# soedinglab/spacedust

Hardware: AMD Instinct MI355X
Metric: clustersearch throughput (genome-pairs/s; SW GCUPS alongside) (higher is better)
Workload: dtype int16

## Files before the change

### spacedust_amd/csrc/hip/sd_sw.hip

```cpp
#include "sd_common.h"
#include <unistd.h>


#include <algorithm>
#include <cmath>
#include <cstring>
#include <memory>
#include <omp.h>
#include <numeric>

#include "../host/sd_host.h"
#include "sd_sw_pk.h"

namespace {

using sdpk::SwTask;

template <int RT>
__global__ void __launch_bounds__(64)
sw_score_kernel(const SwTask *__restrict__ tasks, uint32_t nTasks, const uint8_t *__restrict__ qRes,
                const int8_t *__restrict__ qBias, const uint8_t *__restrict__ tRes, const int8_t *__restrict__ mat,
                int go, int ge, int32_t *__restrict__ out, uint2 *__restrict__ boundary,
                const uint32_t *__restrict__ order ,
                const int8_t *__restrict__ qProf ) {
// ... 804 lines not shown
    }
    SD_HIP(ctx, hipMemcpyAsync(hPin, dOut, (size_t) nSlots * 3 * sizeof(int32_t), hipMemcpyDeviceToHost, ctx->stream));
    SD_HIP(ctx, sdStreamSync(ctx));
    memcpy(hOut.data(), hPin, (size_t) nSlots * 3 * sizeof(int32_t));
    return SD_OK;
}


constexpr uint32_t N_NARROW_CLASSES = 24;
constexpr uint32_t FIRST_NARROW_MULTI = 21;
constexpr uint32_t N_PK_CLASSES = 14;
constexpr uint32_t FIRST_MULTI_PK = 11;
constexpr uint32_t FIRST_WIDE_CLASS = N_NARROW_CLASSES;
constexpr uint32_t FIRST_INT32_CLASS = FIRST_WIDE_CLASS + N_PK_CLASSES;
constexpr uint32_t N_SCORE_CLASSES = FIRST_INT32_CLASS + 4;
static_assert(N_SCORE_CLASSES < 63, "class boundaries are found by one 64-lane wavefront; six class bits in the pair key");
enum ScoreKernel { SCORE_PK = 0, SCORE_PK_WIDE = 1, SCORE_INT32 = 2 };
constexpr uint32_t KEY_INVALID = N_SCORE_CLASSES * 1024u;
__host__ __device__ __forceinline__ bool scoreClassIsMulti(uint32_t ci) {
    return (ci >= FIRST_NARROW_MULTI && ci < FIRST_WIDE_CLASS) || (ci >= FIRST_WIDE_CLASS + FIRST_MULTI_PK && ci < FIRST_INT32_CLASS);
}
__device__ __forceinline__ uint32_t scoreKey(int n, int tL, int kernel, int wideRowLimit = 800) {
    int ci;
    if (kernel == SCORE_PK_WIDE && min(n, tL) > wideRowLimit) kernel = SCORE_INT32;
    if (kernel == SCORE_INT32 || tL > 65535) {
        ci = FIRST_INT32_CLASS + (n <= 128 ? 0 : (n <= 256 ? 1 : (n <= 512 ? 2 : 3)));
    } else if (kernel == SCORE_PK_WIDE) {
        if (n <= 192) ci = n <= 128 ? 0 : 1;
        else if (n <= 384) ci = 2 + (n - 193) / 32;
        else if (n <= 768) ci = n <= 512 ? 8 : (n <= 640 ? 9 : 10);
        else ci = min((int) FIRST_MULTI_PK + (n + 511) / 512 - 2, 13);
        ci += FIRST_WIDE_CLASS;
    } else {
        if (n <= 128) ci = 0;
        else if (n <= 768) ci = (n + 31) / 32 - 4;
        else ci = min((int) FIRST_NARROW_MULTI + (n + 511) / 512 - 2, (int) FIRST_WIDE_CLASS - 1);
    }
    return (uint32_t) ci * 1024u + (uint32_t) (1023 - min(tL >> 4, 1023));
}

struct DevGateParams {
    int go, ge, matMin, swMode, covMode, wideRowLimit;
    float covThr;
    double evalThr;
    double lambda, K, aI, bI, alphaI, betaI, aJ, bJ, alphaJ, betaJ, sigma, tau, viThr, vjThr, cThr, dbResidues;
};

__device__ double devEvalue(const DevGateParams &e, double y_, double qLen) {
    const double m_ = e.dbResidues, n_ = qLen;
    const double const_val = 0.3989422804014327;
    double tmp = e.aI * y_ + e.bI;
    double m_li_y = m_ - tmp;
    double vi_y = fmax(e.viThr, e.alphaI * y_ + e.betaI);
    double sqrt_vi_y = sqrt(vi_y);
    double m_F = sqrt_vi_y == 0.0 ? 1e100 : m_li_y / sqrt_vi_y;
    double P_m_F = 0.5 * erfc(-sqrt(0.5) * m_F);
    double E_m_F = -const_val * exp(-0.5 * m_F * m_F);
    double p1 = m_li_y * P_m_F - sqrt_vi_y * E_m_F;
    tmp = e.aJ * y_ + e.bJ;
    double n_lj_y = n_ - tmp;
    double vj_y = fmax(e.vjThr, e.alphaJ * y_ + e.betaJ);
    double sqrt_vj_y = sqrt(vj_y);
    double n_F = sqrt_vj_y == 0.0 ? 1e100 : n_lj_y / sqrt_vj_y;
    double P_n_F = 0.5 * erfc(-sqrt(0.5) * n_F);
    double E_n_F = -const_val * exp(-0.5 * n_F * n_F);
    double p2 = n_lj_y * P_n_F - sqrt_vj_y * E_n_F;
    double c_y = fmax(e.cThr, e.sigma * y_ + e.tau);
    double area = p1 * p2 + c_y * (P_m_F * P_n_F);
    return e.K * exp(-e.lambda * y_) * area;
}

__device__ __forceinline__ float devCov(unsigned int startPos, unsigned int endPos, unsigned int len) {
    return (min(len, max(startPos, endPos)) - min(startPos, endPos) + 1) / (float) len;
}
__device__ __forceinline__ bool devHasCoverage(float covThr, int covMode, float qCov, float tCov) {
    switch (covMode) {
        case 0: return (qCov >= covThr) && (tCov >= covThr);
        case 2: return qCov >= covThr;
        case 1: return tCov >= covThr;
        default: return true;
    }
}

__global__ void __launch_bounds__(256)
k_pre_word(uint32_t nPairs, const uint32_t *__restrict__ pairQ, const uint32_t *__restrict__ pairT, const uint16_t *__restrict__ pairDiag,
           const uint32_t *__restrict__ fwdKeys, const uint64_t *__restrict__ qOff, const uint64_t *__restrict__ tOff,
           const uint8_t *__restrict__ qRes, const int8_t *__restrict__ qBias, const uint8_t *__restrict__ tRes, const int8_t *__restrict__ mat,
           const int8_t *__restrict__ qProf, const int32_t *__restrict__ minBias, int matMin, uint8_t *__restrict__ preWord,
           uint32_t *__restrict__ pass1Keys) {
    __shared__ int8_t smat[441];
    for (int x = threadIdx.x; x < 441; x += blockDim.x) smat[x] = mat[x];
    __syncthreads();
    const uint32_t i = blockIdx.x * blockDim.x + threadIdx.x;
    if (i >= nPairs) return;
    uint8_t pw = 0;
    const uint32_t key = fwdKeys[i];
    if (key != KEY_INVALID) {
        const uint64_t qo = qOff[pairQ[i]], to = tOff[pairT[i]];
        const int qL = (int) (qOff[pairQ[i] + 1] - qo), tL = (int) (tOff[pairT[i] + 1] - to);
        if (qL < 32768 && tL < 32768 && pairDiag[i] != 0x8000) {
            const int d = (int) (int16_t) pairDiag[i];
            int q0 = d >= 0 ? d : 0, t0 = d >= 0 ? 0 : -d;
            const int n = min(qL - q0, tL - t0);
            const int need = 255 - (abs(matMin) + abs(minBias[pairQ[i]]));
            int run = 0, best = 0;
            for (int x = 0; x < n && best < need; x++) {
                const int qr = qRes[qo + q0 + x], tr = tRes[to + t0 + x];
                run += qProf ? (int) qProf[(qo + q0 + x) * 21 + tr] : (int) smat[tr * 21 + qr] + (int) qBias[qo + q0 + x];
                run = run < 0 ? 0 : run;
                best = run > best ? run : best;
            }
            pw = best >= need ? 1 : 0;
        }
    }
    preWord[i] = pw;
    pass1Keys[i] = pw ? KEY_INVALID : key;
}

__global__ void __launch_bounds__(256)
k_make_fwd(uint32_t nPairs, const uint32_t *__restrict__ pairQ, const uint32_t *__restrict__ pairT,
           const uint8_t *__restrict__ ident, const uint64_t *__restrict__ qOff, const uint64_t *__restrict__ tOff,
           SwTask *__restrict__ tasks, uint32_t *__restrict__ keys, uint32_t *__restrict__ vals,
           sd_sw_result *__restrict__ res, int usePk) {
    const uint32_t i = blockIdx.x * blockDim.x + threadIdx.x;
    if (i >= nPairs) return;
    const uint64_t qo = qOff[pairQ[i]], to = tOff[pairT[i]];
    const int qL = (int) (qOff[pairQ[i] + 1] - qo), tL = (int) (tOff[pairT[i] + 1] - to);
    SwTask tk;
    tk.qOff = qo; tk.tOff = to; tk.n = qL; tk.tL = tL; tk.qStep = 1; tk.tStep = 1;
    tk.segLen = max(1, (qL + 31) / 32);
    tk.slot = i; tk.boundOff = 0;
    const bool valid = !(ident && ident[i]) && qL > 0 && tL > 0;
    tasks[i] = tk;
    keys[i] = valid ? scoreKey(qL, tL, usePk ? SCORE_PK : SCORE_INT32) : KEY_INVALID;
    vals[i] = i;
    sd_sw_result r;
    r.score = 0; r.qStart = -1; r.qEnd = -1; r.tStart = -1; r.tEnd = -1; r.identical = 0; r.btLen = 0; r.flags = 0;
    r.evalue = 0.0; r.btOffset = 0;
    res[i] = r;
}

__global__ void k_bounds(const uint32_t *__restrict__ keys, uint32_t n, uint32_t step, uint32_t *__restrict__ b, int nb) {
    const int c = threadIdx.x;
    if (c >= nb) return;
    const uint64_t want = (uint64_t) c * step;
    uint32_t lo = 0, hi = n;
    while (lo < hi) {
        uint32_t mid = (lo + hi) >> 1;
        if ((uint64_t) keys[mid] < want) lo = mid + 1;
        else hi = mid;
    }
    b[c] = lo;
}

__global__ void __launch_bounds__(256)
k_gate_word(uint32_t nPairs, const uint32_t *__restrict__ pairQ, const int32_t *__restrict__ out32,
            const int32_t *__restrict__ minBias, int matMin, SwTask *__restrict__ tasks, uint32_t *__restrict__ keys,
            uint32_t *__restrict__ vals, uint8_t *__restrict__ word, const uint32_t *__restrict__ fwdKeys, int usePk, int wideRowLimit,
            const uint8_t *__restrict__ preWord ) {
    const uint32_t i = blockIdx.x * blockDim.x + threadIdx.x;
    if (i >= nPairs) return;
    vals[i] = i;
    bool w = false;
    if (fwdKeys[i] != KEY_INVALID) {
        const int mb = minBias[pairQ[i]];
        const int bias = abs(matMin) + abs(mb);
        w = (preWord && preWord[i]) || out32[3 * i] + bias >= 255;
    }
    word[i] = w ? 1 : 0;
    if (w) {
        tasks[i].segLen = max(1, (tasks[i].n + 15) / 16);
        keys[i] = scoreKey(tasks[i].n, tasks[i].tL, usePk ? SCORE_PK_WIDE : SCORE_INT32, wideRowLimit);
    } else {
        keys[i] = KEY_INVALID;
    }
}

__global__ void __launch_bounds__(256)
k_gate_rev(uint32_t nPairs, DevGateParams gp, const uint32_t *__restrict__ pairQ, const uint32_t *__restrict__ pairT,
           const uint64_t *__restrict__ qOff, const uint64_t *__restrict__ tOff, const int32_t *__restrict__ out32,
           const int32_t *__restrict__ out16, const uint8_t *__restrict__ word, const uint32_t *__restrict__ fwdKeys,
           SwTask *__restrict__ tasks, uint32_t *__restrict__ keys, uint32_t *__restrict__ vals,
           sd_sw_result *__restrict__ res, int usePk) {
    const uint32_t i = blockIdx.x * blockDim.x + threadIdx.x;
    if (i >= nPairs) return;
    vals[i] = i;
    keys[i] = KEY_INVALID;
    if (fwdKeys[i] == KEY_INVALID) return;
    const int32_t *src = word[i] ? &out16[3 * i] : &out32[3 * i];
    sd_sw_result r = res[i];
    r.score = src[0];
    r.tEnd = src[1];
    r.qEnd = src[2];
    r.flags = word[i] ? 1 : 0;
    if (word[i] && r.tEnd == -1) r.tEnd = 0;
    if (r.score == 0) r.qEnd = 0;
    if (r.tEnd == -1) { res[i] = r; return; }
    const uint64_t qo = qOff[pairQ[i]], to = tOff[pairT[i]];
    const int qL = (int) (qOff[pairQ[i] + 1] - qo), tL = (int) (tOff[pairT[i] + 1] - to);
// ... 918 lines not shown
    std::unique_ptr<HostScope> hs(new HostScope(ctx, "align.upload"));
    DevGateParams gp;
    gp.go = go; gp.ge = ge; gp.matMin = matMin; gp.swMode = par->swMode; gp.covMode = par->covMode; gp.covThr = par->covThr;
    {
        int matMax = 0;
        for (int x = 0; x < 441; x++) matMax = std::max(matMax, (int) par->matrix[x]);
        const int maxEntry = std::max(1, queries->dProf ? queries->maxEntryAdd : matMax + queries->maxEntryAdd);
        gp.wideRowLimit = 32767 / maxEntry;
    }
    gp.evalThr = par->evalThr;
    gp.lambda = ev.lambda; gp.K = ev.K; gp.aI = ev.aI; gp.bI = ev.bI; gp.alphaI = ev.alphaI; gp.betaI = ev.betaI;
    gp.aJ = ev.aJ; gp.bJ = ev.bJ; gp.alphaJ = ev.alphaJ; gp.betaJ = ev.betaJ; gp.sigma = ev.sigma; gp.tau = ev.tau;
    gp.viThr = ev.viThr; gp.vjThr = ev.vjThr; gp.cThr = ev.cThr; gp.dbResidues = ev.dbResidues;

    const size_t N = nPairs;
    const unsigned grid = (unsigned) ((N + 255) / 256);
    int8_t *dMat = nullptr;
    uint32_t *dPQ = nullptr, *dPT = nullptr, *dKeys = nullptr, *dVals = nullptr, *dKeysS = nullptr, *dOrder = nullptr,
             *dBounds = nullptr, *dFwdKeys = nullptr, *dRevKeys = nullptr;
    uint8_t *dIdent = nullptr, *dWord = nullptr;
    int32_t *dMinBias = nullptr, *dOut32 = nullptr, *dOut16 = nullptr, *dOutRev = nullptr, *dTbRes = nullptr;
    int *dErr = nullptr;
    SwTask *dTasks = nullptr;
    TbTask *dTb = nullptr;
    sd_sw_result *dRes = nullptr;
    uint64_t *dScanA = nullptr, *dScanB = nullptr, *dDirBytes = nullptr, *dDirOff = nullptr, *dBtBytes = nullptr,
             *dBtOff = nullptr, *dBtLen = nullptr, *dDense = nullptr;
    unsigned long long *dCells = nullptr;
    SD_HIP(ctx, wsGet(ctx, "al.mat", 448, &dMat));
    SD_HIP(ctx, wsGet(ctx, "al.pq", N, &dPQ));
    SD_HIP(ctx, wsGet(ctx, "al.pt", N, &dPT));
    SD_HIP(ctx, wsGet(ctx, "al.ident", N, &dIdent));
    SD_HIP(ctx, wsGet(ctx, "al.word", N, &dWord));
    SD_HIP(ctx, wsGet(ctx, "al.keys", N, &dKeys));
    SD_HIP(ctx, wsGet(ctx, "al.vals", N, &dVals));
    SD_HIP(ctx, wsGet(ctx, "al.keyss", N, &dKeysS));
    SD_HIP(ctx, wsGet(ctx, "al.order", N, &dOrder));
    SD_HIP(ctx, wsGet(ctx, "al.fwdkeys", N, &dFwdKeys));
    SD_HIP(ctx, wsGet(ctx, "al.revkeys", N, &dRevKeys));
    SD_HIP(ctx, wsGet(ctx, "al.bounds", 64, &dBounds));
    SD_HIP(ctx, wsGet(ctx, "al.minbias", queries->n, &dMinBias));
    SD_HIP(ctx, wsGet(ctx, "al.out32", N * 3, &dOut32));
    SD_HIP(ctx, wsGet(ctx, "al.out16", N * 3, &dOut16));
    SD_HIP(ctx, wsGet(ctx, "al.outrev", N * 3, &dOutRev));
    SD_HIP(ctx, wsGet(ctx, "al.tbres", N * 2, &dTbRes));
    SD_HIP(ctx, wsGet(ctx, "al.err", 4, &dErr));
    SD_HIP(ctx, wsGet(ctx, "al.tasks", N, &dTasks));
    SD_HIP(ctx, wsGet(ctx, "al.tb", N, &dTb));
    SD_HIP(ctx, wsGet(ctx, "al.res", N, &dRes));
    ctx->alignDevRes = dRes;
    ctx->alignDevResN = N;
    SD_HIP(ctx, wsGet(ctx, "al.scana", N + 1, &dScanA));
    SD_HIP(ctx, wsGet(ctx, "al.scanb", N + 1, &dScanB));
    SD_HIP(ctx, wsGet(ctx, "al.dirbytes", N + 1, &dDirBytes));
    SD_HIP(ctx, wsGet(ctx, "al.diroff", N + 1, &dDirOff));
    SD_HIP(ctx, wsGet(ctx, "al.btbytes", N + 1, &dBtBytes));
    SD_HIP(ctx, wsGet(ctx, "al.btoff", N + 1, &dBtOff));
    SD_HIP(ctx, wsGet(ctx, "al.btlen", N + 1, &dBtLen));
    SD_HIP(ctx, wsGet(ctx, "al.dense", N + 1, &dDense));
    SD_HIP(ctx, wsGet(ctx, "al.cells", 4, &dCells));
    SD_HIP(ctx, hipMemcpyAsync(dMat, par->matrix, 441, hipMemcpyHostToDevice, ctx->stream));
    SD_HIP(ctx, hipMemcpyAsync(dPQ, pairQ, N * sizeof(uint32_t), hipMemcpyHostToDevice, ctx->stream));
    SD_HIP(ctx, hipMemcpyAsync(dPT, pairT, N * sizeof(uint32_t), hipMemcpyHostToDevice, ctx->stream));
    if (isIdentity) SD_HIP(ctx, hipMemcpyAsync(dIdent, isIdentity, N, hipMemcpyHostToDevice, ctx->stream));
    else SD_HIP(ctx, hipMemsetAsync(dIdent, 0, N, ctx->stream));
    SD_HIP(ctx, hipMemcpyAsync(dMinBias, queries->dProf ? queries->hProfBias.data() : queries->hMinBias.data(),
                               queries->n * sizeof(int32_t), hipMemcpyHostToDevice, ctx->stream));
    SD_HIP(ctx, hipMemsetAsync(dErr, 0, 4 * sizeof(int), ctx->stream));
    SD_HIP(ctx, hipMemsetAsync(dCells, 0, 4 * sizeof(unsigned long long), ctx->stream));
    SD_HIP(ctx, hipMemsetAsync(dOut32, 0, N * 3 * sizeof(int32_t), ctx->stream));
    SD_HIP(ctx, hipMemsetAsync(dOut16, 0, N * 3 * sizeof(int32_t), ctx->stream));
    SD_HIP(ctx, hipMemsetAsync(dOutRev, 0, N * 3 * sizeof(int32_t), ctx->stream));
    SD_HIP(ctx, hipMemsetAsync(dBtLen, 0, (N + 1) * sizeof(uint64_t), ctx->stream));

    hs.reset(new HostScope(ctx, "align.fwd32"));
    const int usePk = (go >= ge && go < 1024 && ge >= 0 && getenv("SD_SW_INT32") == nullptr) ? 1 : 0;
    uint32_t nValid = 0;
    hipLaunchKernelGGL(k_make_fwd, dim3(grid), dim3(256), 0, ctx->stream, nPairs, dPQ, dPT, dIdent, queries->dOff, targets->dOff,
                       dTasks, dFwdKeys, dVals, dRes, usePk);
    uint32_t *dPass1Keys = dFwdKeys;
    uint8_t *dPreWord = nullptr;
    if (pairDiag && usePk) {
        uint16_t *dDiag = nullptr;
        SD_HIP(ctx, wsGet(ctx, "al.diag", N, &dDiag));
        SD_HIP(ctx, wsGet(ctx, "al.preword", N, &dPreWord));
        SD_HIP(ctx, wsGet(ctx, "al.pass1keys", N, &dPass1Keys));
        SD_HIP(ctx, hipMemcpyAsync(dDiag, pairDiag, N * sizeof(uint16_t), hipMemcpyHostToDevice, ctx->stream));
        hipLaunchKernelGGL(k_pre_word, dim3(grid), dim3(256), 0, ctx->stream, nPairs, (const uint32_t *) dPQ, (const uint32_t *) dPT,
                           (const uint16_t *) dDiag, (const uint32_t *) dFwdKeys, (const uint64_t *) queries->dOff, (const uint64_t *) targets->dOff,
                           (const uint8_t *) queries->dRes, (const int8_t *) queries->dBias, (const uint8_t *) targets->dRes, (const int8_t *) dMat,
                           (const int8_t *) queries->dProf, (const int32_t *) dMinBias, queries->dProf ? 0 : matMin, dPreWord, dPass1Keys);
    }
    hipLaunchKernelGGL(k_cells, dim3(grid), dim3(256), 0, ctx->stream, nPairs, dTasks, dPass1Keys, dCells + 0);
    const uint32_t *dShare = queries->n >= (1u << PAIR_QUERY_BITS) ? nullptr : dPQ;
    int rc = devRunScore(ctx, nPairs, dPass1Keys, dVals, dKeysS, dOrder, dBounds, dTasks, dScanA, dScanB, queries, targets, dMat, go,
                         ge, dOut32, &nValid, dShare);
    if (rc != SD_OK) return rc;
    hs.reset(new HostScope(ctx, "align.fwd16"));
    hipLaunchKernelGGL(k_gate_word, dim3(grid), dim3(256), 0, ctx->stream, nPairs, dPQ, dOut32, dMinBias, queries->dProf ? 0 : matMin, dTasks, dKeys,
                       dVals, dWord, dFwdKeys, usePk, gp.wideRowLimit, (const uint8_t *) dPreWord);
    hipLaunchKernelGGL(k_cells, dim3(grid), dim3(256), 0, ctx->stream, nPairs, dTasks, dKeys, dCells + 0);
    rc = devRunScore(ctx, nPairs, dKeys, dVals, dKeysS, dOrder, dBounds, dTasks, dScanA, dScanB, queries, targets, dMat, go, ge,
                     dOut16, &nValid, dShare);
    if (rc != SD_OK) return rc;
    hs.reset(new HostScope(ctx, "align.rev"));
    hipLaunchKernelGGL(k_gate_rev, dim3(grid), dim3(256), 0, ctx->stream, nPairs, gp, dPQ, dPT, queries->dOff, targets->dOff, dOut32,
                       dOut16, dWord, dFwdKeys, dTasks, dRevKeys, dVals, dRes, usePk);
    hipLaunchKernelGGL(k_cells, dim3(grid), dim3(256), 0, ctx->stream, nPairs, dTasks, dRevKeys, dCells + 1);
    rc = devRunScore(ctx, nPairs, dRevKeys, dVals, dKeysS, dOrder, dBounds, dTasks, dScanA, dScanB, queries, targets, dMat, go, ge,
                     dOutRev, &nValid, nullptr);
    if (rc != SD_OK) return rc;
    hs.reset(new HostScope(ctx, "align.traceback"));
    hipLaunchKernelGGL(k_gate_tb, dim3(grid), dim3(256), 0, ctx->stream, nPairs, gp, dPQ, dPT, queries->dOff, targets->dOff, dOutRev,
                       dRevKeys, dTb, dKeys, dVals, dDirBytes, dBtBytes, dRes, dErr);
    SD_HIP(ctx, hipMemsetAsync(dBtBytes + N, 0, sizeof(uint64_t), ctx->stream));
    rc = devExclusiveScan(ctx, dBtBytes, dBtOff, N + 1);
    if (rc != SD_OK) return rc;
    uint64_t btScratch = 0;
    SD_HIP(ctx, sdD2H(ctx, &btScratch, dBtOff + N, sizeof(uint64_t)));
    SD_HIP(ctx, sdStreamSync(ctx));
    char *dBt = nullptr;
    SD_HIP(ctx, wsGet(ctx, "tb.bt", btScratch + 64, &dBt));
    uint64_t SCRATCH_BUDGET = 16ull << 30;
    {
        size_t freeB = 0, totalB = 0;
        if (hipMemGetInfo(&freeB, &totalB) == hipSuccess && totalB > 0)
            SCRATCH_BUDGET = std::max<uint64_t>(1ull << 30, std::min<uint64_t>(totalB / 4, freeB / 3));
        if (const char *e = getenv("SD_TB_BUDGET")) SCRATCH_BUDGET = std::max<uint64_t>(1u << 20, strtoull(e, nullptr, 10));
    }
    uint32_t *dKeysRound = nullptr;
    SD_HIP(ctx, wsGet(ctx, "tb.keysRound", N + 1, &dKeysRound));
    bool tbPending = false, budgetRaised = false;
    for (int round = 0; round < 4096; round++) {
        tbPending = true;
        SD_HIP(ctx, hipMemsetAsync(dDirBytes + N, 0, sizeof(uint64_t), ctx->stream));
        rc = devExclusiveScan(ctx, dDirBytes, dDirOff, N + 1);
        if (rc != SD_OK) return rc;
        hipLaunchKernelGGL(k_tb_round, dim3(grid), dim3(256), 0, ctx->stream, nPairs, dKeys, dDirOff, dDirBytes, SCRATCH_BUDGET, dKeysRound);
        hipLaunchKernelGGL(k_tb_offsets, dim3(grid), dim3(256), 0, ctx->stream, nPairs, dKeysRound, dDirOff, dBtOff, dTb);
        rc = devSortPairs(ctx, dKeysRound, dKeysS, dVals, dOrder, nPairs, 16);
        if (rc != SD_OK) return rc;
        hipLaunchKernelGGL(k_bounds, dim3(1), dim3(64), 0, ctx->stream, dKeysS, nPairs, 4096u, dBounds, (int) N_TB_CLASSES + 1);
        uint32_t hb[N_TB_CLASSES + 1];
        uint64_t dirTotal = 0;
        SD_HIP(ctx, sdD2H(ctx, hb, dBounds, sizeof(hb)));
        SD_HIP(ctx, sdD2H(ctx, &dirTotal, dDirOff + N, sizeof(uint64_t)));
        SD_HIP(ctx, sdStreamSync(ctx));
        if (hb[N_TB_CLASSES] == 0) {
            if (dirTotal == 0) {
                tbPending = false;
                break;
            }
            if (SCRATCH_BUDGET >= dirTotal) return sdFail(ctx, SD_EHIP, "traceback: pending tasks but an empty round (budget %llu, pending %llu bytes)",
                                                          (unsigned long long) SCRATCH_BUDGET, (unsigned long long) dirTotal);
            SCRATCH_BUDGET = std::min<uint64_t>(dirTotal, SCRATCH_BUDGET * 2);
            budgetRaised = true;
            continue;
        }
        if (getenv("SD_DEBUG_TB")) {
            fprintf(stderr, "[tb] round %d: narrow", round);
            for (int ci = 0; ci < N_TB_NARROW; ci++) fprintf(stderr, " %u", hb[ci + 1] - hb[ci]);
            fprintf(stderr, " lds %u %u %u global %u dir %.1f MB\n", hb[N_TB_NARROW + 1] - hb[N_TB_NARROW], hb[N_TB_NARROW + 2] - hb[N_TB_NARROW + 1],
                    hb[N_TB_NARROW + 3] - hb[N_TB_NARROW + 2], hb[N_TB_NARROW + 4] - hb[N_TB_NARROW + 3], dirTotal / 1e6);
        }
        int8_t *dDir = nullptr;
        if (wsGet(ctx, "tb.dir", std::min<uint64_t>(dirTotal, SCRATCH_BUDGET) + 64, &dDir) != hipSuccess) {
            (void) hipGetLastError();
            if (SCRATCH_BUDGET <= (256ull << 20) || budgetRaised)
                return sdFail(ctx, SD_ENOMEM, "traceback direction scratch: out of device memory (%llu bytes for one round)",
                              (unsigned long long) std::min<uint64_t>(dirTotal, SCRATCH_BUDGET));
            SCRATCH_BUDGET /= 2;
            continue;
        }
        for (int ci = 0; ci < N_TB_NARROW; ci++) {
            const uint32_t begin = hb[ci], cnt = hb[ci + 1] - hb[ci];
            if (cnt == 0) continue;
            static const char *const tbNames[N_TB_NARROW] = {"sw_traceback.narrow128", "sw_traceback.narrow192", "sw_traceback.narrow256",
                                                             "sw_traceback.narrow320", "sw_traceback.narrow384", "sw_traceback.narrow512",
                                                             "sw_traceback.narrow640", "sw_traceback.narrow768", "sw_traceback.narrow1024"};
            ProfScope ps(ctx, tbNames[ci]);
            const int qCap = TB_NARROW_Q[ci], tCap = qCap + 16;
            const size_t ldsBytes = 2 * ((size_t) 16 * qCap + 2 * (size_t) qCap + tCap);
            if (queries->dProf)
                hipLaunchKernelGGL(sw_traceback_narrow_kernel<true>, dim3((cnt + 1) / 2), dim3(64), ldsBytes, ctx->stream, dTb, cnt,
// ... 604 lines not shown
```

### spacedust_amd/csrc/host/sd_search.cpp

```cpp
#include "sd_host.h"
#include "sd_target_build.h"
#include "spacedust_gpu.h"

#include <algorithm>
#include <chrono>
#include <condition_variable>
#include <cstdio>
#include <cstdlib>
#include <cstring>
#include <deque>
#include <fstream>
#include <functional>
#include <future>
#include <memory>
#include <mutex>
#include <string>
#include <thread>
#include <pthread.h>
#include <vector>

namespace {

double nowSec() {
    return std::chrono::duration<double>(std::chrono::steady_clock::now().time_since_epoch()).count();
// ... 516 lines not shown
        const uint64_t r0 = Q->offsets[c0], r1 = Q->offsets[c1];
        o->off.resize((size_t) nq + 1);
        for (uint32_t i = 0; i <= nq; i++) o->off[i] = Q->offsets[c0 + i] - r0;
        if (profile) {
            o->cpu = threadCpuSec() - cpu0;
            return o;
        }
        const double t0 = nowSec();
        o->sw.assign(r1 - r0 + 1, 0);
        if (s->ungapped) {
            if (s->par.compBiasCorr) o->rc = sd_host_sw_comp_bias(s->host, 0, Q->residues + r0, o->off.data(), nq, o->sw.data());
            o->seconds = nowSec() - t0;
            o->cpu = threadCpuSec() - cpu0;
            return o;
        }
        o->dg.assign(r1 - r0 + 1, 0);
        o->km.assign(r1 - r0 + 1, 0);
        if (s->par.compBiasCorr) {
            if (s->ctxBias)
                o->rc = sd_comp_bias_batch(s->ctxBias, s->host, Q->residues + r0, o->off.data(), nq, s->k, o->sw.data(), o->dg.data(), o->km.data());
            else
                o->rc = sd_host_comp_bias(s->host, Q->residues + r0, o->off.data(), nq, s->k, o->sw.data(), o->dg.data(), o->km.data());
        }
        o->seconds = nowSec() - t0;
        o->cpu = threadCpuSec() - cpu0;
        return o;
    };
    typedef std::future<std::unique_ptr<BiasOut> > BiasFut;
    auto pfJob = [s, Q, profile, sameDb](std::shared_ptr<BiasFut> bf, sd_ctx *pfCtx) {
        std::unique_ptr<PfOut> o(new PfOut());
        o->bias = bf->get();
        const double cpu0 = threadCpuSec();
        BiasOut &b = *o->bias;
        if (b.rc != SD_OK) {
            o->rc = b.rc;
            o->err = "composition bias";
            return o;
        }
        const uint32_t nq = b.c1 - b.c0;
        const uint64_t r0 = Q->offsets[b.c0];
        std::vector<uint32_t> ident(nq);
        for (uint32_t i = 0; i < nq; i++) ident[i] = sameDb ? b.c0 + i : UINT32_MAX;
        const uint32_t W = (uint32_t) s->pfPar.maxHitsPerQuery;
        o->hits.resize((size_t) nq * W);
        o->counts.assign(nq, 0);
        o->stats.assign((size_t) nq * 4, 0);
        double t0 = nowSec();
        if (s->ungapped) {
            sd_seqset *qs = nullptr;
            o->rc = sd_seqset_create(pfCtx, Q->residues + r0, b.off.data(), nq, s->par.compBiasCorr ? b.sw.data() : nullptr, &qs);
            if (o->rc == SD_OK) {
                o->rc = sd_ungapped_prefilter_batch(pfCtx, &s->ugPar, qs, s->tSeqs, s->T.keys, ident.data(), o->hits.data(), o->counts.data());
                sd_seqset_destroy(qs);
            }
        } else if (profile)
            o->rc = sd_prefilter_profile_batch(pfCtx, s->target, &s->pfPar, nq, Q->residues + r0, b.off.data(), Q->sortedScore + r0 * 20,
                                               Q->sortedIndex + r0 * 20, Q->alnProfile + r0 * 21, ident.data(), o->hits.data(),
                                               o->counts.data(), o->stats.data());
        else
            o->rc = sd_prefilter_batch(pfCtx, s->target, &s->pfPar, nq, Q->residues + r0, b.off.data(), b.km.data(), b.dg.data(),
                                       ident.data(), o->hits.data(), o->counts.data(), o->stats.data());
        o->tPrefilter = nowSec() - t0;
        if (o->rc != SD_OK) {
            o->err = std::string(s->ungapped ? "sd_ungapped_prefilter_batch: " : "sd_prefilter_batch: ") + sd_last_error(pfCtx);
            return o;
        }
        for (uint32_t i = 0; i < nq; i++)
            if (o->counts[i] == UINT32_MAX) {
                o->counts[i] = 0;
                if (!o->notComputed) o->err = sd_last_error(pfCtx);
                o->notComputed++;
            }
        t0 = nowSec();
        o->nPairs = sd_host_pair_list(o->hits.data(), o->counts.data(), nq, W, nullptr, nullptr);
        o->pairQ.resize(std::max<uint64_t>(o->nPairs, 1));
        o->pairT.resize(std::max<uint64_t>(o->nPairs, 1));
        if (o->nPairs) sd_host_pair_list(o->hits.data(), o->counts.data(), nq, W, o->pairQ.data(), o->pairT.data());
        o->pairDiag.resize(std::max<uint64_t>(o->nPairs, 1));
        {
            uint64_t w = 0;
            for (uint32_t q = 0; q < nq; q++) {
                const sd_hit *row = o->hits.data() + (size_t) q * W;
                for (uint32_t x = 0; x < o->counts[q]; x++)
                    o->pairDiag[w++] = (row[x].score >= 200 && !s->ungapped) ? row[x].diagonal : (uint16_t) 0x8000;
            }
        }
        o->tPairs = nowSec() - t0;
        o->cpu = threadCpuSec() - cpu0;
        return o;
    };
    typedef std::future<std::unique_ptr<PfOut> > PfFut;
    std::vector<std::shared_ptr<BiasFut> > biasFut(chunks.size());
    auto submitBias = [&](size_t x) {
        if (x < chunks.size() && !biasFut[x]) {
            const uint32_t c0 = chunks[x].c0, c1 = chunks[x].c1;
            biasFut[x].reset(new BiasFut(biasStage.submit([biasJob, c0, c1] { return biasJob(c0, c1); })));
        }
    };
    const int pfLanes = s->pfLanes;
    std::unique_ptr<StageThread> pfLaneMore[3];
    for (int l = 1; l < pfLanes; l++) pfLaneMore[l - 1].reset(new StageThread(("sd-pf" + std::to_string(l)).c_str()));
    sd_ctx *pfCtxOf[4] = {s->ctxPf, s->ctxPf2, s->ctxPfMore[0], s->ctxPfMore[1]};
    auto submitPf = [&](size_t x) {
        submitBias(x);
        std::shared_ptr<BiasFut> bf = biasFut[x];
        sd_ctx *pfCtx = pfCtxOf[x % (size_t) pfLanes];
        StageThread &st = (x % (size_t) pfLanes) ? *pfLaneMore[x % (size_t) pfLanes - 1] : pfStage;
        PfFut f = st.submit([pfJob, bf, pfCtx] { return pfJob(bf, pfCtx); });
        for (int a = 1; a <= pfLanes; a++) submitBias(x + (size_t) a);
        return f;
    };

    int status = SD_OK;
    StageThread finStage{"sd-fin"};
    std::mutex finMu;
    std::future<std::pair<int, double> > pending;
    std::unique_ptr<double> aggCpu(new double(0.0));
    double *aggCpuP = aggCpu.get();
    const double mainCpu0 = threadCpuSec();
    bool havePending = false;
    size_t pendingChunk = 0;
    auto waitPending = [&]() {
        if (!havePending) return;
        const double t0 = nowSec();
        const std::pair<int, double> r = pending.get();
        {
            std::lock_guard<std::mutex> l(finMu);
            tm[T_AGG_WAIT] += nowSec() - t0;
        }
        tm[T_AGG_BUSY] += r.second;
        havePending = false;
        if (r.first != SD_OK && status == SD_OK) status = s->fail(r.first, "sd_agg_add");
    };

    auto finalize = [&](uint32_t r, std::string *errOut) -> int {
        auto failF = [&](int rc_, const std::string &what, sd_ctx *ctx_ = nullptr) {
            *errOut = what + " failed (" + std::to_string(rc_) + ")";
            if (ctx_) *errOut += std::string(": ") + sd_last_error(ctx_);
            return rc_;
        };
        double tAggWait = 0, tCh = 0;
        struct Clocks {
            std::mutex &m;
            double *tm;
            double &a, &c;
            ~Clocks() {
                std::lock_guard<std::mutex> l(m);
                tm[T_AGG_WAIT] += a;
                tm[T_CLUSTERHITS] += c;
            }
        } clocks{finMu, tm, tAggWait, tCh};
        sd_search_result &R = *res[r];
        if (!aggregate) return SD_OK;
        double t0 = nowSec();
        uint64_t ne = 0, nh = 0;
        int rc = sd_agg_finish(R.agg, &ne, &nh);
        if (rc != SD_OK) return failF(rc, "sd_agg_finish");
        R.entryOff.assign(ne + 1, 0);
        R.entryQ.assign(std::max<uint64_t>(ne, 1), 0);
        R.entryT.assign(std::max<uint64_t>(ne, 1), 0);
        R.hitQ.assign(std::max<uint64_t>(nh, 1), 0);
        R.hitT.assign(std::max<uint64_t>(nh, 1), 0);
        R.pval.assign(std::max<uint64_t>(nh, 1), 0.0);
        rc = sd_agg_get(R.agg, R.entryOff.data(), R.entryQ.data(), R.entryT.data(), R.hitQ.data(), R.hitT.data(), R.pval.data());
        if (rc != SD_OK) return failF(rc, "sd_agg_get");
        R.entryQ.resize(ne);
        R.entryT.resize(ne);
// ... 370 lines not shown
```

Before: 2902.

## Add banded gapped pre-check to skip full int32 SW for near-saturating pairs

Pairs whose ungapped diagonal score falls short of the saturation threshold but exceeds a gate are compacted via a scan and re-scored with a 33-wide banded gapped Smith-Waterman around the prefilter diagonal. If the banded score reaches the saturation bound, the pair is marked as word-saturating and dropped from the first full scoring pass. The host also lowers the prefilter score threshold for supplying diagonals, so more pairs get the pre-check. This adds a scan, a compaction kernel and the banded kernel, plus an optional debug stats dump.

```diff
diff --git a/spacedust_amd/csrc/hip/sd_sw.hip b/spacedust_amd/csrc/hip/sd_sw.hip
--- a/spacedust_amd/csrc/hip/sd_sw.hip
+++ b/spacedust_amd/csrc/hip/sd_sw.hip
@@ -910,18 +910,20 @@
     }
 }
 
+constexpr int PW_BAND = 16;
+constexpr int PW_GATE = 90;
 __global__ void __launch_bounds__(256)
 k_pre_word(uint32_t nPairs, const uint32_t *__restrict__ pairQ, const uint32_t *__restrict__ pairT, const uint16_t *__restrict__ pairDiag,
            const uint32_t *__restrict__ fwdKeys, const uint64_t *__restrict__ qOff, const uint64_t *__restrict__ tOff,
            const uint8_t *__restrict__ qRes, const int8_t *__restrict__ qBias, const uint8_t *__restrict__ tRes, const int8_t *__restrict__ mat,
            const int8_t *__restrict__ qProf, const int32_t *__restrict__ minBias, int matMin, uint8_t *__restrict__ preWord,
-           uint32_t *__restrict__ pass1Keys) {
+           uint32_t *__restrict__ pass1Keys, uint8_t *__restrict__ cand) {
     __shared__ int8_t smat[441];
     for (int x = threadIdx.x; x < 441; x += blockDim.x) smat[x] = mat[x];
     __syncthreads();
     const uint32_t i = blockIdx.x * blockDim.x + threadIdx.x;
     if (i >= nPairs) return;
-    uint8_t pw = 0;
+    uint8_t pw = 0, cd = 0;
     const uint32_t key = fwdKeys[i];
     if (key != KEY_INVALID) {
         const uint64_t qo = qOff[pairQ[i]], to = tOff[pairT[i]];
@@ -939,10 +941,78 @@
                 best = run > best ? run : best;
             }
             pw = best >= need ? 1 : 0;
+            cd = (!pw && best >= PW_GATE) ? 1 : 0;
         }
     }
     preWord[i] = pw;
     pass1Keys[i] = pw ? KEY_INVALID : key;
+    cand[i] = cd;
+}
+__global__ void __launch_bounds__(256)
+k_pre_word_list(uint32_t nPairs, const uint8_t *__restrict__ cand, const uint64_t *__restrict__ pos, uint32_t *__restrict__ list) {
+    const uint32_t i = blockIdx.x * blockDim.x + threadIdx.x;
+    if (i < nPairs && cand[i]) list[pos[i]] = i;
+}
+constexpr int PW_OUT = 1 << 20;
+template <bool PROF>
+__global__ void __launch_bounds__(256)
+k_pre_word_band(uint32_t nPairs, const uint64_t *__restrict__ pos, const uint32_t *__restrict__ list, const uint32_t *__restrict__ pairQ,
+                const uint32_t *__restrict__ pairT, const uint16_t *__restrict__ pairDiag, const uint64_t *__restrict__ qOff,
+                const uint64_t *__restrict__ tOff, const uint8_t *__restrict__ qRes, const int8_t *__restrict__ qBias,
+                const uint8_t *__restrict__ tRes, const int8_t *__restrict__ mat, const int8_t *__restrict__ qProf,
+                const int32_t *__restrict__ minBias, int matMin, int go, int ge, uint8_t *__restrict__ preWord, uint32_t *__restrict__ pass1Keys) {
+    constexpr int BAND = PW_BAND, W = 2 * BAND + 1;
+    const uint64_t nCand = pos[nPairs];
+    if ((uint64_t) blockIdx.x * blockDim.x >= nCand) return;
+    __shared__ int8_t smat[441];
+    for (int x = threadIdx.x; x < 441; x += blockDim.x) smat[x] = mat[x];
+    __syncthreads();
+    const uint32_t x = blockIdx.x * blockDim.x + threadIdx.x;
+    if ((uint64_t) x >= nCand) return;
+    const uint32_t i = list[x];
+    const uint64_t qo = qOff[pairQ[i]], to = tOff[pairT[i]];
+    const int qL = (int) (qOff[pairQ[i] + 1] - qo), tL = (int) (tOff[pairT[i] + 1] - to);
+    const int d = (int) (int16_t) pairDiag[i];
+    const int need = 255 - (abs(matMin) + abs(minBias[pairQ[i]]));
+    const int c0 = max(0, -d - BAND), c1 = min(tL - 1, qL - 1 - d + BAND);
+    auto rowInfo = [&](int q) -> int {
+        if (q < 0 || q >= qL) return PROF ? -1 : (int) ((uint32_t) -PW_OUT << 8);
+        return PROF ? q : ((int) qRes[qo + q] | (int) ((uint32_t) (int) qBias[qo + q] << 8));
+    };
+    int G[W], E[W + 1], QI[W];
+#pragma unroll
+    for (int k = 0; k < W; k++) {
+        G[k] = 0;
+        E[k] = 0;
+        QI[k] = rowInfo(c0 - 1 + d - BAND + k);
+    }
+    E[W] = 0;
+    int best = 0;
+    for (int c = c0; c <= c1 && best < need; c++) {
+        const int tr = tRes[to + c];
+        const int qNew = rowInfo(c + d + BAND);
+        int F = 0;
+#pragma unroll
+        for (int k = 0; k < W; k++) {
+            const int qi = k + 1 < W ? QI[k + 1] : qNew;
+            QI[k] = qi;
+            int P;
+            if (PROF) P = qi < 0 ? -PW_OUT : (int) qProf[(qo + (uint64_t) qi) * 21 + tr];
+            else P = (int) smat[tr * 21 + (qi & 0xFF)] + (qi >> 8);
+            const int e = E[k + 1];
+            const int hpre = max(max(G[k] + P, e), 0);
+            const int g = max(hpre, F);
+            const int open = hpre - go;
+            E[k] = max(e - ge, open);
+            F = max(F - ge, open);
+            G[k] = g;
+            best = max(best, g);
+        }
+    }
+    if (best >= need) {
+        preWord[i] = 1;
+        pass1Keys[i] = KEY_INVALID;
+    }
 }
 
 __global__ void __launch_bounds__(256)
@@ -2027,14 +2097,38 @@
     uint8_t *dPreWord = nullptr;
     if (pairDiag && usePk) {
         uint16_t *dDiag = nullptr;
+        uint8_t *dCand = nullptr;
+        uint64_t *dCandPos = nullptr;
+        uint32_t *dCandList = nullptr;
         SD_HIP(ctx, wsGet(ctx, "al.diag", N, &dDiag));
         SD_HIP(ctx, wsGet(ctx, "al.preword", N, &dPreWord));
         SD_HIP(ctx, wsGet(ctx, "al.pass1keys", N, &dPass1Keys));
+        SD_HIP(ctx, wsGet(ctx, "al.pwcand", N + 1, &dCand));
+        SD_HIP(ctx, wsGet(ctx, "al.pwpos", N + 1, &dCandPos));
+        SD_HIP(ctx, wsGet(ctx, "al.pwlist", N, &dCandList));
         SD_HIP(ctx, hipMemcpyAsync(dDiag, pairDiag, N * sizeof(uint16_t), hipMemcpyHostToDevice, ctx->stream));
-        hipLaunchKernelGGL(k_pre_word, dim3(grid), dim3(256), 0, ctx->stream, nPairs, (const uint32_t *) dPQ, (const uint32_t *) dPT,
-                           (const uint16_t *) dDiag, (const uint32_t *) dFwdKeys, (const uint64_t *) queries->dOff, (const uint64_t *) targets->dOff,
-                           (const uint8_t *) queries->dRes, (const int8_t *) queries->dBias, (const uint8_t *) targets->dRes, (const int8_t *) dMat,
-                           (const int8_t *) queries->dProf, (const int32_t *) dMinBias, queries->dProf ? 0 : matMin, dPreWord, dPass1Keys);
+        SD_HIP(ctx, hipMemsetAsync(dCand + N, 0, 1, ctx->stream));
+        const int pwMatMin = queries->dProf ? 0 : matMin;
+        {
+            ProfScope ps(ctx, "sw_pre_word");
+            hipLaunchKernelGGL(k_pre_word, dim3(grid), dim3(256), 0, ctx->stream, nPairs, (const uint32_t *) dPQ, (const uint32_t *) dPT,
+                               (const uint16_t *) dDiag, (const uint32_t *) dFwdKeys, (const uint64_t *) queries->dOff, (const uint64_t *) targets->dOff,
+                               (const uint8_t *) queries->dRes, (const int8_t *) queries->dBias, (const uint8_t *) targets->dRes, (const int8_t *) dMat,
+                               (const int8_t *) queries->dProf, (const int32_t *) dMinBias, pwMatMin, dPreWord, dPass1Keys, dCand);
+        }
+        ProfScope psb(ctx, "sw_pre_word.band");
+        const int rcS = devExclusiveScan(ctx, (const uint8_t *) dCand, dCandPos, N + 1);
+        if (rcS != SD_OK) return rcS;
+        hipLaunchKernelGGL(k_pre_word_list, dim3(grid), dim3(256), 0, ctx->stream, nPairs, (const uint8_t *) dCand, (const uint64_t *) dCandPos, dCandList);
+#define SD_PW_BAND_LAUNCH(PROF)                                                                                                                \
+    hipLaunchKernelGGL(k_pre_word_band<PROF>, dim3(grid), dim3(256), 0, ctx->stream, nPairs, (const uint64_t *) dCandPos,                      \
+                       (const uint32_t *) dCandList, (const uint32_t *) dPQ, (const uint32_t *) dPT, (const uint16_t *) dDiag,                 \
+                       (const uint64_t *) queries->dOff, (const uint64_t *) targets->dOff, (const uint8_t *) queries->dRes,                    \
+                       (const int8_t *) queries->dBias, (const uint8_t *) targets->dRes, (const int8_t *) dMat, (const int8_t *) queries->dProf, \
+                       (const int32_t *) dMinBias, pwMatMin, go, ge, dPreWord, dPass1Keys)
+        if (queries->dProf) SD_PW_BAND_LAUNCH(true);
+        else SD_PW_BAND_LAUNCH(false);
+#undef SD_PW_BAND_LAUNCH
     }
     hipLaunchKernelGGL(k_cells, dim3(grid), dim3(256), 0, ctx->stream, nPairs, dTasks, dPass1Keys, dCells + 0);
     const uint32_t *dShare = queries->n >= (1u << PAIR_QUERY_BITS) ? nullptr : dPQ;
@@ -2045,6 +2139,22 @@
     hipLaunchKernelGGL(k_gate_word, dim3(grid), dim3(256), 0, ctx->stream, nPairs, dPQ, dOut32, dMinBias, queries->dProf ? 0 : matMin, dTasks, dKeys,
                        dVals, dWord, dFwdKeys, usePk, gp.wideRowLimit, (const uint8_t *) dPreWord);
     hipLaunchKernelGGL(k_cells, dim3(grid), dim3(256), 0, ctx->stream, nPairs, dTasks, dKeys, dCells + 0);
+    if (getenv("SD_DEBUG_PW")) {
+        std::vector<uint8_t> hW(nPairs), hP(nPairs, 0);
+        std::vector<SwTask> hT(nPairs);
+        SD_HIP(ctx, hipStreamSynchronize(ctx->stream));
+        SD_HIP(ctx, hipMemcpy(hW.data(), dWord, nPairs, hipMemcpyDeviceToHost));
+        if (dPreWord) SD_HIP(ctx, hipMemcpy(hP.data(), dPreWord, nPairs, hipMemcpyDeviceToHost));
+        SD_HIP(ctx, hipMemcpy(hT.data(), dTasks, (size_t) nPairs * sizeof(SwTask), hipMemcpyDeviceToHost));
+        unsigned long long nW = 0, nP = 0, cW = 0, cP = 0, cAll = 0;
+        for (uint32_t i = 0; i < nPairs; i++) {
+            const unsigned long long c = (unsigned long long) hT[i].n * (unsigned long long) hT[i].tL;
+            cAll += c;
+            if (hW[i]) { nW++; cW += c; }
+            if (hW[i] && hP[i]) { nP++; cP += c; }
+        }
+        fprintf(stderr, "[pw] pairs %u word %llu skipped %llu cells_all %llu cells_word %llu cells_skipped %llu\n", nPairs, nW, nP, cAll, cW, cP);
+    }
     rc = devRunScore(ctx, nPairs, dKeys, dVals, dKeysS, dOrder, dBounds, dTasks, dScanA, dScanB, queries, targets, dMat, go, ge,
                      dOut16, &nValid, dShare);
     if (rc != SD_OK) return rc;
diff --git a/spacedust_amd/csrc/host/sd_search.cpp b/spacedust_amd/csrc/host/sd_search.cpp
--- a/spacedust_amd/csrc/host/sd_search.cpp
+++ b/spacedust_amd/csrc/host/sd_search.cpp
@@ -622,7 +622,7 @@
             for (uint32_t q = 0; q < nq; q++) {
                 const sd_hit *row = o->hits.data() + (size_t) q * W;
                 for (uint32_t x = 0; x < o->counts[q]; x++)
-                    o->pairDiag[w++] = (row[x].score >= 200 && !s->ungapped) ? row[x].diagonal : (uint16_t) 0x8000;
+                    o->pairDiag[w++] = (row[x].score >= 60 && !s->ungapped) ? row[x].diagonal : (uint16_t) 0x8000;
             }
         }
         o->tPairs = nowSec() - t0;
```

New measurement: 2886 (median of 2 runs). Within noise of the previous version (-0.6%).
